# Lakonik/SSDNeRF

Measured on NVIDIA H100. Metric: rays/sec (128^2 render) & DDIM triplanes/sec, higher is better.
Workload: dtype fp16 tensor-core UNet (fp32 accumulate), fp32 renderer

## Files before the change

### ssdnerf_b200/csrc/conv_row2.cu

```cuda
#include "common.cuh"
#include "tc_common.cuh"
#include "conv_row_epilogue.cuh"
#include "../../include/ssdnerf_b200.h"
#include <cuda_fp16.h>

namespace ssdnerf {
using namespace tc;

constexpr int kRwThreads = 384;
constexpr int kRwRowSlot = 17 * 1024;
constexpr int kRwBSlot = kRwN * 128;
constexpr int kRwRows = 6, kRwBStages = 6;
constexpr int kGnMaxC = 384;
constexpr size_t kRwSmem = (size_t)kRwRows * kRwRowSlot + (size_t)kRwBStages * kRwBSlot + 1024  + 256  +
                           256  + 512 ;

struct ConvRowParams {
    uint32_t B, H;
    const __half* x1; uint32_t C1;
    const __half* x2; uint32_t C2;
    long long xs1[3], xs2[3];
    const float2* coef;
    const float* bias;
    const __half* residual;
    __half* out;
    float* qstats;
};

template <bool GN>
__global__ void __launch_bounds__(kRwThreads, 1)
k_conv_row2(const __grid_constant__ CUtensorMap mapB, const ConvRowParams p) {
    extern __shared__ uint8_t smem_raw[];
    uint8_t* smem = reinterpret_cast<uint8_t*>(((uintptr_t)smem_raw + 1023) & ~(uintptr_t)1023);
    uint8_t* sR = smem;
    uint8_t* sB = smem + kRwRows * kRwRowSlot;
    uint64_t* fullR = reinterpret_cast<uint64_t*>(sB + kRwBStages * kRwBSlot);
    uint64_t* emptyR = fullR + kRwRows;
    uint64_t* fullB = emptyR + kRwRows;
    uint64_t* emptyB = fullB + kRwBStages;
    float* qacc = reinterpret_cast<float*>(reinterpret_cast<uint8_t*>(fullR) + 256);
    float* sbias = qacc + 64;

    const int warp = threadIdx.x >> 5, lane = threadIdx.x & 31, wg = warp >> 2;
    const uint32_t tiles_per_img = p.H / 2, total_tiles = p.B * tiles_per_img;
    const uint32_t kc1 = p.C1 / 64, KC = (p.C1 + p.C2) / 64;
    const uint32_t tile0 = blockIdx.x, tstep = gridDim.x;
    const uint32_t my_tiles = tile0 < total_tiles ? (total_tiles - tile0 + tstep - 1) / tstep : 0;

    if (threadIdx.x == 0) {
        prefetch_tmap(&mapB);
        for (int i = 0; i < kRwRows; ++i) { mbar_init(&fullR[i], 4); mbar_init(&emptyR[i], 8); }
        for (int i = 0; i < kRwBStages; ++i) { mbar_init(&fullB[i], 1); mbar_init(&emptyB[i], 8); }
        fence_mbar_init();
    }
    for (int i = threadIdx.x; i < 64; i += kRwThreads) qacc[i] = 0.0f;
    for (int i = threadIdx.x; i < kRwN; i += kRwThreads) sbias[i] = p.bias ? __ldg(p.bias + i) : 0.0f;
    __syncthreads();
    pdl_trigger();
    pdl_wait();

    if (wg == 2) {
        setmaxnreg_dec<120>();
        const uint32_t lt = threadIdx.x - 256u;
        const uint32_t c8 = lt & 7u, p0 = lt >> 3;
        const uint32_t C = p.C1 + p.C2;
        uint32_t idx = 0;
        for (uint32_t tile = tile0; tile < total_tiles; tile += tstep) {
            const uint32_t b = tile / tiles_per_img, y0 = (tile - b * tiles_per_img) * 2;
            for (uint32_t j = 0; j < KC; ++j) {
                const bool first = j < kc1;
                const __half* src = first ? p.x1 : p.x2;
                const long long xs0 = first ? p.xs1[0] : p.xs2[0], xs1 = first ? p.xs1[1] : p.xs2[1], xs2 = first ? p.xs1[2] : p.xs2[2];
                const uint32_t cl = (first ? j : j - kc1) * 64u + c8 * 8u;
                float ca[8], cb[8];
                if (GN) {
                    const float4* cp = reinterpret_cast<const float4*>(p.coef + (size_t)b * C + j * 64u + c8 * 8u);
#pragma unroll
                    for (int k = 0; k < 4; ++k) {
                        const float4 t = __ldg(cp + k);
                        ca[2 * k] = 0.5f * t.x; cb[2 * k] = 0.5f * t.y; ca[2 * k + 1] = 0.5f * t.z; cb[2 * k + 1] = 0.5f * t.w;
                    }
                }
                for (uint32_t r = 0; r < 4; ++r) {
                    const int y = (int)(y0 + r) - 1;
                    const bool row_ok = y >= 0 && y < (int)p.H;
                    const __half* rowp = src + (long long)b * xs2 + (long long)(row_ok ? y : 0) * xs1 + cl;
                    uint4 v[9];
#pragma unroll
                    for (int n = 0; n < 9; ++n) {
                        const int x = (int)(p0 + 16u * n) - 1;
                        v[n] = (row_ok && (unsigned)x < (unsigned)kRwW) ? __ldg(reinterpret_cast<const uint4*>(rowp + (long long)x * xs0))
                                                                       : make_uint4(0, 0, 0, 0);
                    }
                    const uint32_t slot = idx % kRwRows;
                    mbar_wait(&emptyR[slot], ((idx / kRwRows) & 1u) ^ 1u);
                    const uint32_t dst = smem_u32(sR + slot * kRwRowSlot);
#pragma unroll
                    for (int n = 0; n < 9; ++n) {
                        const uint32_t px = p0 + 16u * n;
                        if (px >= 130u) continue;
                        uint4 o = v[n];
                        if (GN) {
                            const bool ok = row_ok && (unsigned)((int)px - 1) < (unsigned)kRwW;
                            const __half2* h = reinterpret_cast<const __half2*>(&v[n]);
                            uint32_t* ow = reinterpret_cast<uint32_t*>(&o);
#pragma unroll
                            for (int k = 0; k < 4; ++k) {
                                const float2 tt = __half22float2(h[k]);
                                const __half2 hh = __floats2half2_rn(fmaf(tt.x, ca[2 * k], cb[2 * k]), fmaf(tt.y, ca[2 * k + 1], cb[2 * k + 1]));
                                uint32_t hv = *reinterpret_cast<const uint32_t*>(&hh), tv;
                                asm("tanh.approx.f16x2 %0, %1;" : "=r"(tv) : "r"(hv));
                                const __half2 yy = __hfma2(hh, *reinterpret_cast<const __half2*>(&tv), hh);
                                ow[k] = ok ? *reinterpret_cast<const uint32_t*>(&yy) : 0u;
                            }
                        }
                        sts128(dst + px * 128u + ((c8 ^ (px & 7u)) << 4), o);
                    }
                    __syncwarp();
                    if (lane == 0) mbar_arrive(&fullR[slot]);
                    ++idx;
                }
            }
        }
    } else {
        setmaxnreg_inc<192>();
        const uint32_t a = (uint32_t)wg, wq = (uint32_t)warp & 3u, cq = (uint32_t)lane & 3u;
        const uint32_t steps_per_tile = KC * 9u, total_steps = my_tiles * steps_per_tile;
        auto issue_w = [&](uint32_t L) {
            const uint32_t s = L % kRwBStages;
            if (L >= (uint32_t)kRwBStages) mbar_wait(&emptyB[s], ((L / kRwBStages) - 1u) & 1u);
            mbar_expect_tx(&fullB[s], (uint32_t)kRwBSlot);
            const uint32_t rem = L % steps_per_tile;
            tma_load_4d(sB + s * kRwBSlot, &mapB, &fullB[s], (int)((rem / 9u) * 64u), 0, (int)(rem % 9u), 0);
        };
        if (threadIdx.x == 0)
            for (uint32_t L = 0; L < total_steps && L < (uint32_t)kRwBStages; ++L) issue_w(L);
        auto release_row = [&](uint32_t ring) { if (lane == 0) mbar_arrive(&emptyR[ring % kRwRows]); };
        uint32_t m = 0, ridx = 0;
        const uint32_t lrow = wq * 16u + ((uint32_t)lane & 15u);
        const uint32_t lk = (uint32_t)lane >> 4;
        for (uint32_t tile = tile0; tile < total_tiles; tile += tstep) {
            const uint32_t b = tile / tiles_per_img, y0 = (tile - b * tiles_per_img) * 2;
            float acc0[64], acc1[64];
#pragma unroll
            for (int i = 0; i < 64; ++i) { acc0[i] = 0.0f; acc1[i] = 0.0f; }
            for (uint32_t j = 0; j < KC; ++j) {
                const uint32_t unused = ridx + (a == 0 ? 3u : 0u);
                if (a == 1) { mbar_wait(&fullR[unused % kRwRows], (unused / kRwRows) & 1u); release_row(unused); }
                for (uint32_t ky = 0; ky < 3; ++ky) {
                    const uint32_t ring = ridx + ky + a;
                    mbar_wait(&fullR[ring % kRwRows], (ring / kRwRows) & 1u);
                    const uint32_t rowS = smem_u32(sR + (ring % kRwRows) * kRwRowSlot);
                    for (uint32_t kx = 0; kx < 3; ++kx) {
                        const uint32_t sb = m % kRwBStages;
                        uint32_t af[2][4][4];
#pragma unroll
                        for (uint32_t h = 0; h < 2; ++h) {
                            const uint32_t px = 64u * h + lrow + kx;
#pragma unroll
                            for (uint32_t k = 0; k < 4; ++k) ldmatrix_x4(rowS + px * 128u + (((2u * k + lk) ^ (px & 7u)) << 4), af[h][k]);
                        }
                        if (kx == 2) release_row(ring);
                        mbar_wait(&fullB[sb], (m / kRwBStages) & 1u);
                        const uint64_t b_desc = make_desc_sw128(smem_u32(sB + sb * kRwBSlot));
                        wgmma_fence();
                        fence_regs(acc0); fence_regs(acc1);
#pragma unroll
                        for (uint32_t k = 0; k < 4; ++k) {
                            wgmma_rs_n128(acc0, af[0][k], b_desc + 2 * k, 1u);
                            wgmma_rs_n128(acc1, af[1][k], b_desc + 2 * k, 1u);
                        }
                        wgmma_commit();
                        wgmma_wait<0>();
                        fence_regs(acc0); fence_regs(acc1);
                        if (lane == 0) mbar_arrive(&emptyB[sb]);
                        if (threadIdx.x == 0 && m >= 1 && m - 1 + kRwBStages < total_steps) issue_w(m - 1 + kRwBStages);
                        ++m;
                    }
                }
                if (a == 0) { mbar_wait(&fullR[unused % kRwRows], (unused / kRwRows) & 1u); release_row(unused); }
                ridx += 4;
            }
            const size_t pix0 = ((size_t)b * p.H + y0 + a) * kRwW;
#pragma unroll
            for (int i = 0; i < 16; ++i) {
                const uint32_t ch = 8u * i + 2u * cq;
                const float b0 = sbias[ch], b1 = sbias[ch + 1];
                float su = 0.0f, sq = 0.0f;
#pragma unroll
                for (int h = 0; h < 2; ++h) {
#pragma unroll
                    for (int hh = 0; hh < 2; ++hh) {
                        const size_t o = (pix0 + 64u * h + wq * 16u + ((uint32_t)lane >> 2) + 8u * hh) * kRwN + ch;
                        float v0 = (h ? acc1 : acc0)[4 * i + 2 * hh] + b0, v1 = (h ? acc1 : acc0)[4 * i + 2 * hh + 1] + b1;
                        if (p.residual) { const float2 r = __half22float2(*reinterpret_cast<const __half2*>(p.residual + o)); v0 += r.x; v1 += r.y; }
                        *reinterpret_cast<__half2*>(p.out + o) = __floats2half2_rn(v0, v1);
                        su += v0 + v1; sq = fmaf(v0, v0, fmaf(v1, v1, sq));
                    }
                }
                if (p.qstats) {
                    frag_quad_reduce(su, sq);
                    if ((lane & ~2) == 0) { float* qa = qacc + (2 * i + (lane >> 1)) * 2; atomicAdd(qa, su); atomicAdd(qa + 1, sq); }
                }
            }
            if (p.qstats) {
                asm volatile("bar.sync 1, 256;" ::: "memory");
                if (threadIdx.x < 64) {
                    const float val = qacc[threadIdx.x];
                    if (val != 0.0f) atomicAdd(p.qstats + (size_t)b * 64 + threadIdx.x, val);
                    qacc[threadIdx.x] = 0.0f;
                }
                asm volatile("bar.sync 1, 256;" ::: "memory");
            }
        }
    }
    __syncthreads();
}

__global__ void k_gn_coef(const float* __restrict__ q1, uint32_t C1, const float* __restrict__ q2, uint32_t C2, uint32_t HW,
                          const float* __restrict__ gamma, const float* __restrict__ beta, const float* __restrict__ scale_shift,
                          long long ss_batch_stride, float eps, float2* __restrict__ coef) {
    pdl_trigger();
    pdl_wait();
    __shared__ float2 s_mr[32];
    const uint32_t b = blockIdx.x, C = C1 + C2, cpg = C / 32u;
    const float inv_n = 1.0f / ((float)HW * (float)cpg);
    if (threadIdx.x < 32u) {
        const uint32_t q1n = C1 / 4, q2n = C2 / 4, nq = cpg / 4;
        float sm = 0.0f, sq = 0.0f;
        for (uint32_t i = 0; i < nq; ++i) {
            const uint32_t qi = threadIdx.x * nq + i;
            const float2 t = __ldg(reinterpret_cast<const float2*>(qi < q1n ? q1 + ((size_t)b * q1n + qi) * 2 : q2 + ((size_t)b * q2n + (qi - q1n)) * 2));
            sm += t.x; sq += t.y;
        }
        const float mean = sm * inv_n;
        s_mr[threadIdx.x] = make_float2(mean, rsqrtf(fmaxf(sq * inv_n - mean * mean, 0.0f) + eps));
    }
    __syncthreads();
    const float* ss = scale_shift ? scale_shift + (size_t)b * ss_batch_stride : nullptr;
    for (uint32_t c = threadIdx.x; c < C; c += blockDim.x) {
        const float2 mr = s_mr[c / cpg];
        const float ak = mr.y * __ldg(gamma + c);
        const float bk = __ldg(beta + c) - mr.x * ak;
        const float sc = ss ? 1.0f + __ldg(ss + c) : 1.0f, sh = ss ? __ldg(ss + C + c) : 0.0f;
        coef[(size_t)b * C + c] = make_float2(ak * sc, fmaf(bk, sc, sh));
    }
}

int make_map_4d_box(CUtensorMap* m, const void* base, uint64_t K, uint64_t e1, uint64_t e2, uint64_t e3, uint64_t s1, uint64_t s2, uint64_t s3,
                    uint32_t x1, uint32_t x2, uint32_t x3);

template <bool GN>
static int launch_row2(const CUtensorMap& mB, const ConvRowParams& p, int sms, cudaStream_t stream) {
    static DeviceOnce attr;
    if (attr.first()) {
        SSDNERF_CUDA_OK(cudaFuncSetAttribute(k_conv_row2<GN>, cudaFuncAttributeMaxDynamicSharedMemorySize, (int)kRwSmem));
    }
    const uint32_t total = p.B * (p.H / 2);
    SSDNERF_CUDA_OK(launch_pdl(k_conv_row2<GN>, dim3(total < (uint32_t)sms ? total : (uint32_t)sms), dim3(kRwThreads), kRwSmem, stream, mB, p));
    SSDNERF_LAUNCH_OK();
    return 0;
}

int conv_row2_launch(const ssdnerf_gemm_args* a, int sms, cudaStream_t stream) {
    if (((uintptr_t)a->a1 & 15u) || ((a->a1_strides[0] | a->a1_strides[1] | a->a1_strides[2]) & 15u) ||
        (a->a2 && (((uintptr_t)a->a2 & 15u) || ((a->a2_strides[0] | a->a2_strides[1] | a->a2_strides[2]) & 15u))) ||
        ((uintptr_t)a->out & 3u) || ((uintptr_t)a->residual & 3u))
        return set_error_msg(SSDNERF_ERR_ARG, "gemm: row-pair convolution needs 16-byte aligned inputs and strides, 4-byte aligned output / residual");
    ConvRowParams p{};
    p.B = a->d3; p.H = a->d2;
    p.x1 = (const __half*)a->a1; p.C1 = a->k1;
    p.x2 = (const __half*)a->a2; p.C2 = a->a2 ? a->k2 : 0;
    for (int i = 0; i < 3; ++i) { p.xs1[i] = (long long)(a->a1_strides[i] / 2); p.xs2[i] = a->a2 ? (long long)(a->a2_strides[i] / 2) : 0; }
    p.bias = a->bias_n; p.residual = (const __half*)a->residual; p.out = (__half*)a->out; p.qstats = a->qstats;
    const uint64_t ktot = (uint64_t)a->k1 + (a->a2 ? a->k2 : 0);
    CUtensorMap mB;
    if (int e = make_map_4d_box(&mB, a->b, ktot, a->n_rows_b ? a->n_rows_b : a->n, a->bx2 ? a->bx2 : 1, a->bx3 ? a->bx3 : 1, a->b_strides[0],
                                a->b_strides[1], a->b_strides[2], kRwN, 1, 1)) return e;
    return launch_row2<false>(mB, p, sms, stream);
}

}

using namespace ssdnerf;

extern "C" int ssdnerf_conv3x3_gn_f16(const ssdnerf_conv_gn_args* a, void* stream_) {
    cudaStream_t stream = (cudaStream_t)stream_;
    if (!a || !a->x1 || !a->q1 || !a->gamma || !a->beta || !a->w || !a->out || !a->coef_workspace)
        return set_error_msg(SSDNERF_ERR_ARG, "conv3x3_gn: x1, q1, gamma, beta, w, out and coef_workspace are required");
    if (a->B == 0 || a->H == 0) return 0;
    if (a->H % 2) return set_error_msg(SSDNERF_ERR_ARG, "conv3x3_gn: H must be even (tiles are row pairs)");
    if (a->C1 == 0 || a->C1 % 64 || a->C2 % 64 || (a->x2 && !a->q2)) return set_error_msg(SSDNERF_ERR_ARG, "conv3x3_gn: channel counts must be multiples of 64; x2 needs q2");
    const uint32_t C = a->C1 + (a->x2 ? a->C2 : 0);
    if (C > (uint32_t)kGnMaxC || (C / 32) % 4) return set_error_msg(SSDNERF_ERR_ARG, "conv3x3_gn: at most 384 input channels, channels per group a multiple of 4");
    if (a->w_rows < 128) return set_error_msg(SSDNERF_ERR_ARG, "conv3x3_gn: packed weight needs >= 128 rows per tap");
    if (((uintptr_t)a->x1 | (uintptr_t)a->x2 | (uintptr_t)a->out | (uintptr_t)a->residual | (uintptr_t)a->w | (uintptr_t)a->coef_workspace) & 15u)
        return set_error_msg(SSDNERF_ERR_ARG, "conv3x3_gn: tensors must be 16-byte aligned");
    ConvRowParams p{};
    p.B = a->B; p.H = a->H; p.x1 = (const __half*)a->x1; p.C1 = a->C1; p.x2 = (const __half*)a->x2; p.C2 = a->x2 ? a->C2 : 0;
    p.xs1[0] = p.C1; p.xs1[1] = (long long)kRwW * p.C1; p.xs1[2] = (long long)p.H * kRwW * p.C1;
    p.xs2[0] = p.C2; p.xs2[1] = (long long)kRwW * p.C2; p.xs2[2] = (long long)p.H * kRwW * p.C2;
    p.coef = (const float2*)a->coef_workspace; p.bias = a->bias; p.residual = (const __half*)a->residual; p.out = (__half*)a->out; p.qstats = a->qstats;
    int dev = 0, sms = 0;
    SSDNERF_CUDA_OK(cudaGetDevice(&dev));
    SSDNERF_CUDA_OK(cudaDeviceGetAttribute(&sms, cudaDevAttrMultiProcessorCount, dev));
    SSDNERF_CUDA_OK(launch_pdl(k_gn_coef, dim3(a->B), dim3(128), 0, stream, a->q1, a->C1, a->x2 ? a->q2 : (const float*)nullptr, p.C2, a->H * 128u,
                               a->gamma, a->beta, a->scale_shift, a->ss_batch_stride, a->eps, (float2*)a->coef_workspace));
    SSDNERF_LAUNCH_OK();
    CUtensorMap mB;
    if (int e = make_map_4d_box(&mB, a->w, C, a->w_rows, 9, 1, (uint64_t)C * 2, (uint64_t)a->w_rows * C * 2, (uint64_t)9 * a->w_rows * C * 2,
                                kRwN, 1, 1)) return e;
    return launch_row2<true>(mB, p, sms, stream);
}
```

### ssdnerf_b200/csrc/conv_row_epilogue.cuh

```cuda
#pragma once
#include "common.cuh"

namespace ssdnerf {

constexpr int kRwW = 128, kRwN = 128;

__device__ __forceinline__ void frag_quad_reduce(float& su, float& sq) {
    su += __shfl_xor_sync(0xffffffffu, su, 1); sq += __shfl_xor_sync(0xffffffffu, sq, 1);
#pragma unroll
    for (int m = 4; m <= 16; m <<= 1) { su += __shfl_xor_sync(0xffffffffu, su, m); sq += __shfl_xor_sync(0xffffffffu, sq, m); }
}

}
```

### ssdnerf_b200/csrc/gemm_tc.cu

```cuda
#include "common.cuh"
#include "tc_common.cuh"
#include "conv_row_epilogue.cuh"
#include "../../include/ssdnerf_b200.h"
#include <cuda_fp16.h>
#include <cstdio>

namespace ssdnerf {
using namespace tc;

constexpr int kGemmThreads = 384;
constexpr int kMaxBiasN = 2048;
constexpr int kBM = 128, kBK = 64;
constexpr int kABytes = kBM * kBK * 2;

struct GemmParams {
    uint32_t b1, b2, b3;
    uint32_t d1, d2, d3;
    uint32_t T1, T2, T3;
    uint32_t tiles_n;
    uint32_t taps;
    int8_t tap_ox[9], tap_oy[9];
    uint32_t a_stride;
    uint32_t kc1, kc2;
    uint32_t n_valid;
// ... 169 lines not shown
                        }
                    }
                    if (p.out_f32) {
                        float* op = reinterpret_cast<float*>(p.out) + o;
                        if (p.vec2 && okc1) *reinterpret_cast<float2*>(op) = make_float2(v0, v1);
                        else { op[0] = v0; if (okc1) op[1] = v1; }
                    } else {
                        __half* op = reinterpret_cast<__half*>(p.out) + o;
                        if (p.vec2 && okc1) *reinterpret_cast<__half2*>(op) = __floats2half2_rn(v0, v1);
                        else { op[0] = __float2half_rn(v0); if (okc1) op[1] = __float2half_rn(v1); }
                    }
                    if (!okc1) v1 = 0.0f;
                    su += v0 + v1; sq = fmaf(v0, v0, fmaf(v1, v1, sq));
                }
                if (p.qstats) {
                    frag_quad_reduce(su, sq);
                    if ((lane & ~2) == 0) {
                        float* qa = qacc + (slot * (BN / 4) + 2 * i + (lane >> 1)) * 2;
                        atomicAdd(qa, su); atomicAdd(qa + 1, sq);
                    }
                }
            }
            if (p.qstats) {
                asm volatile("bar.sync 1, 256;" ::: "memory");
                const uint32_t et = threadIdx.x - 128;
                const uint32_t nq = p.n_valid / 4;
                for (uint32_t i = et; i < (uint32_t)BN; i += 256) {
                    const float val = qacc[i];
                    const uint32_t sl = i / (BN / 2), qd = (i % (BN / 2)) >> 1, st = i & 1u;
                    const uint32_t gq = n_tile * (BN / 4) + qd;
                    if (val != 0.0f && gq < nq) atomicAdd(p.qstats + ((size_t)(img0 + sl) * nq + gq) * 2 + st, val);
                    qacc[i] = 0.0f;
                }
                asm volatile("bar.sync 1, 256;" ::: "memory");
            }
        }
        if (p.prof && threadIdx.x == 128) { atomicAdd(p.prof + 2, (unsigned long long)wf); atomicAdd(p.prof + 4, (unsigned long long)(clock64() - ct0)); }
    }
    __syncthreads();
    if (CL > 1) cluster_sync_all();
}

typedef CUresult (*PFN_encodeTiled)(CUtensorMap*, CUtensorMapDataType, cuuint32_t, void*, const cuuint64_t*, const cuuint64_t*,
                                    const cuuint32_t*, const cuuint32_t*, CUtensorMapInterleave, CUtensorMapSwizzle,
                                    CUtensorMapL2promotion, CUtensorMapFloatOOBfill);

static PFN_encodeTiled get_encode() {
    static PFN_encodeTiled fn = nullptr;
    if (!fn) {
        void* p = nullptr;
        cudaDriverEntryPointQueryResult qres;
        if (cudaGetDriverEntryPoint("cuTensorMapEncodeTiled", &p, cudaEnableDefault, &qres) != cudaSuccess || !p) return nullptr;
        fn = (PFN_encodeTiled)p;
    }
    return fn;
}

static int make_map_4d(CUtensorMap* m, const void* base, uint64_t K, uint64_t e1, uint64_t e2, uint64_t e3, uint64_t s1, uint64_t s2,
                       uint64_t s3, uint32_t x1, uint32_t x2, uint32_t x3, uint32_t trav = 1) {
    PFN_encodeTiled enc = get_encode();
    if (!enc) return set_error_msg(SSDNERF_ERR_CUDA, "cuTensorMapEncodeTiled entry point not found");
    if (((uintptr_t)base & 15u) || (s1 & 15u) || (s2 & 15u) || (s3 & 15u))
        return set_error_msg(SSDNERF_ERR_ARG, "gemm: TMA operands need 16-byte aligned base and strides");
    cuuint64_t dims[4] = {K, e1, e2, e3};
    cuuint64_t strides[3] = {s1, s2, s3};
    cuuint32_t box[4] = {64, x1 * trav, x2 * trav, x3};
    cuuint32_t estr[4] = {1, trav, trav, 1};
    const CUresult r = enc(m, CU_TENSOR_MAP_DATA_TYPE_FLOAT16, 4, const_cast<void*>(base), dims, strides, box, estr,
                           CU_TENSOR_MAP_INTERLEAVE_NONE, CU_TENSOR_MAP_SWIZZLE_128B, CU_TENSOR_MAP_L2_PROMOTION_L2_256B,
                           CU_TENSOR_MAP_FLOAT_OOB_FILL_NONE);
    if (r != CUDA_SUCCESS) {
        char buf[200];
        snprintf(buf, sizeof(buf), "cuTensorMapEncodeTiled failed (%d): dims {%llu,%llu,%llu,%llu} box {64,%u,%u,%u}", (int)r,
                 (unsigned long long)K, (unsigned long long)e1, (unsigned long long)e2, (unsigned long long)e3, x1, x2, x3);
        return set_error_msg(SSDNERF_ERR_CUDA, buf);
    }
    return 0;
}

int make_map_4d_box(CUtensorMap* m, const void* base, uint64_t K, uint64_t e1, uint64_t e2, uint64_t e3, uint64_t s1, uint64_t s2, uint64_t s3,
                    uint32_t x1, uint32_t x2, uint32_t x3) {
    return make_map_4d(m, base, K, e1, e2, e3, s1, s2, s3, x1, x2, x3);
}
int conv_row2_launch(const ssdnerf_gemm_args* a, int sms, cudaStream_t stream);

template <int BN, int CL>
static int launch_gemm(const CUtensorMap& mA1, const CUtensorMap& mA2, const CUtensorMap& mB, const GemmParams& p, int sms,
                       cudaStream_t stream) {
    using Cfg = GemmCfg<BN, CL>;
    static DeviceOnce attr;
    if (attr.first()) {
        SSDNERF_CUDA_OK(cudaFuncSetAttribute(k_gemm_tc<BN, CL>, cudaFuncAttributeMaxDynamicSharedMemorySize, (int)Cfg::kSmem));
    }
    const uint32_t tiles_m = p.T1 * p.T2 * p.T3;
    const uint32_t total = ((tiles_m + CL - 1) / CL) * p.tiles_n;
    cudaLaunchConfig_t cfg{};
    cfg.blockDim = dim3(kGemmThreads);
    cfg.dynamicSmemBytes = Cfg::kSmem;
    cfg.stream = stream;
    cudaLaunchAttribute at[2];
    at[0].id = cudaLaunchAttributeClusterDimension;
    at[0].val.clusterDim.x = CL; at[0].val.clusterDim.y = 1; at[0].val.clusterDim.z = 1;
    at[1].id = cudaLaunchAttributeProgrammaticStreamSerialization;
    at[1].val.programmaticStreamSerializationAllowed = pdl_enabled() ? 1 : 0;
    cfg.attrs = at; cfg.numAttrs = 2;
    static int max_clusters_dev[64] = {};
    int& max_clusters_cached = max_clusters_dev[current_device()];
    if (!max_clusters_cached) {
        max_clusters_cached = sms / CL;
        if (CL > 1) {
            cfg.gridDim = dim3((uint32_t)(sms / CL) * CL);
            int n = 0;
            cfg.numAttrs = 1;
            if (cudaOccupancyMaxActiveClusters(&n, k_gemm_tc<BN, CL>, &cfg) == cudaSuccess && n > 0 && n < max_clusters_cached) max_clusters_cached = n;
            cfg.numAttrs = 2;
            (void)cudaGetLastError();
        }
    }
    const uint32_t max_clusters = (uint32_t)max_clusters_cached;
    const uint32_t clusters = total < max_clusters ? total : max_clusters;
    cfg.gridDim = dim3(clusters * CL);
    SSDNERF_CUDA_OK(cudaLaunchKernelEx(&cfg, k_gemm_tc<BN, CL>, mA1, mA2, mB, p));
    SSDNERF_LAUNCH_OK();
    return 0;
}

}

using namespace ssdnerf;

extern "C" int ssdnerf_gemm_f16(const ssdnerf_gemm_args* a, void* stream_) {
    cudaStream_t stream = (cudaStream_t)stream_;
    if (!a || !a->a1 || !a->b || !a->out) return set_error_msg(SSDNERF_ERR_ARG, "gemm: a1, b and out are required");
    if (a->k1 == 0 || a->k1 % 64 || a->k2 % 64) return set_error_msg(SSDNERF_ERR_ARG, "gemm: K extents must be multiples of 64");
    if (a->b1 * a->b2 * a->b3 != 128) return set_error_msg(SSDNERF_ERR_ARG, "gemm: b1*b2*b3 must be 128");
    if (a->taps < 1 || a->taps > 9) return set_error_msg(SSDNERF_ERR_ARG, "gemm: taps must be in [1, 9]");
    if (a->taps != 1 && a->taps != 9 && !a->tap_offsets) return set_error_msg(SSDNERF_ERR_ARG, "gemm: taps other than 1 / 9 need tap_offsets");
    if (a->taps > 1 && a->b_batched) return set_error_msg(SSDNERF_ERR_ARG, "gemm: conv taps and batched B are exclusive");
    if (a->a_stride > 2) return set_error_msg(SSDNERF_ERR_ARG, "gemm: a_stride must be 0 / 1 / 2");
    const uint32_t a_stride = a->a_stride == 2 ? 2u : 1u;
    if (a_stride == 2 && (a->b1 * 2 > 256 || a->b2 * 2 > 256)) return set_error_msg(SSDNERF_ERR_ARG, "gemm: stride-2 boxes exceed the 256-element TMA limit");
    if (a->n == 0 || a->d1 == 0 || a->d2 == 0 || a->d3 == 0) return 0;
    int dev = 0, sms = 0;
    SSDNERF_CUDA_OK(cudaGetDevice(&dev));
    SSDNERF_CUDA_OK(cudaDeviceGetAttribute(&sms, cudaDevAttrMultiProcessorCount, dev));
    if (a->algo != 1 && a->taps == 9 && !a->tap_offsets && a_stride == 1 && a->d1 == 128 && a->b1 == 128 && a->b2 == 1 && a->b3 == 1 && a->n == 128 && !a->out_f32 && !a->b_batched &&
        (a->d2 % 2) == 0 && a->alpha == 1.0f && (a->bn == 0 || a->bn == 128) && a->cluster <= 1 && a->so1 == 128 && a->so2 == 128 * 128 &&
        a->so3 == (long long)a->d2 * 128 * 128 && (!a->qstats || a->stats_hw == 0) && (a->n_rows_b == 0 || a->n_rows_b >= 128))
        return ssdnerf::conv_row2_launch(a, sms, stream);
    if (a->algo == 2) return set_error_msg(SSDNERF_ERR_ARG, "gemm: algo 2 (row-pair convolution) needs taps 9, 128-pixel rows, 128 output channels, fp16 output");
    int bn = (int)a->bn;
    if (!bn) {
        const uint32_t tiles_m = div_up(a->d1, a->b1) * div_up(a->d2, a->b2) * div_up(a->d3, a->b3);
        double best = 1e30;
        const int cand[3] = {256, 128, 64};
        const double eff[3] = {1.0, 0.80, 0.50};
        for (int i = 0; i < 3; ++i) {
            if (cand[i] > 64 && (uint32_t)cand[i] / 2 >= a->n) continue;
            const uint32_t tiles = tiles_m * div_up(a->n, (uint32_t)cand[i]);
            const double t = (double)div_up(tiles, (uint32_t)sms) * cand[i] / eff[i];
            if (t < best) { best = t; bn = cand[i]; }
        }
    }
    if (bn != 64 && bn != 128 && bn != 256) return set_error_msg(SSDNERF_ERR_ARG, "gemm: bn must be 64, 128 or 256");

    GemmParams p{};
    p.b1 = a->b1; p.b2 = a->b2; p.b3 = a->b3; p.d1 = a->d1; p.d2 = a->d2; p.d3 = a->d3;
    p.T1 = div_up(a->d1, a->b1); p.T2 = div_up(a->d2, a->b2); p.T3 = div_up(a->d3, a->b3);
    p.tiles_n = div_up(a->n, (uint32_t)bn);
    p.a_stride = a_stride;
    for (uint32_t t = 0; t < 9; ++t) {
        if (a->tap_offsets) { p.tap_ox[t] = a->tap_offsets[2 * t]; p.tap_oy[t] = a->tap_offsets[2 * t + 1]; }
        else if (a->taps == 9) { p.tap_ox[t] = (int8_t)((int)(t % 3) - 1); p.tap_oy[t] = (int8_t)((int)(t / 3) - 1); }
        else { p.tap_ox[t] = 0; p.tap_oy[t] = 0; }
    }
    p.taps = a->taps; p.kc1 = a->k1 / 64; p.kc2 = a->a2 ? a->k2 / 64 : 0; p.n_valid = a->n; p.b_batched = a->b_batched;
    p.alpha = a->alpha; p.bias_n = a->bias_n; p.residual = (const __half*)a->residual; p.out = a->out; p.out_f32 = a->out_f32;
    p.so1 = a->so1; p.so2 = a->so2; p.so3 = a->so3;
    p.qstats = a->qstats; p.stats_hw = a->stats_hw; p.prof = (unsigned long long*)a->debug_cycles;
    const uintptr_t pair_align = a->out_f32 ? 8u : 4u;
    p.vec2 = ((a->so1 | a->so2 | a->so3) & 1) == 0 && ((uintptr_t)a->out % pair_align) == 0 && ((uintptr_t)a->residual & 3u) == 0;
    if (a->bias_n && a->n > (uint32_t)kMaxBiasN) return set_error_msg(SSDNERF_ERR_ARG, "gemm: bias vectors longer than 2048 are not supported");
    if (a->qstats && (a->n % 4)) return set_error_msg(SSDNERF_ERR_ARG, "gemm: quad statistics need n % 4 == 0");
    if (a->qstats && !a->stats_hw && a->b3 > 2) return set_error_msg(SSDNERF_ERR_ARG, "gemm: fused quad statistics cover at most 2 images per 128-row tile (b3 <= 2)");
    if (a->qstats && a->stats_hw && (a->stats_hw % 64)) return set_error_msg(SSDNERF_ERR_ARG, "gemm: stats_hw must be a multiple of 64");
    const uint64_t ktot = (uint64_t)a->k1 + (a->a2 ? a->k2 : 0);

    CUtensorMap mA1, mA2, mB;
    const uint64_t e1 = (uint64_t)a->d1 * a_stride, e2 = (uint64_t)a->d2 * a_stride;
    if (int e = make_map_4d(&mA1, a->a1, a->k1, e1, e2, a->d3, a->a1_strides[0], a->a1_strides[1], a->a1_strides[2], a->b1, a->b2, a->b3, a_stride)) return e;
    if (a->a2) {
        if (int e = make_map_4d(&mA2, a->a2, a->k2, e1, e2, a->d3, a->a2_strides[0], a->a2_strides[1], a->a2_strides[2], a->b1, a->b2, a->b3, a_stride)) return e;
    } else {
        mA2 = mA1;
    }
    int cl = 1;
    if ((a->cluster == 2 || a->cluster == 4 || a->cluster == 8) && !a->b_batched && bn >= 128) cl = (int)a->cluster;
    if (int e = make_map_4d(&mB, a->b, ktot, a->n_rows_b ? a->n_rows_b : a->n, a->bx2 ? a->bx2 : 1, a->bx3 ? a->bx3 : 1, a->b_strides[0],
                            a->b_strides[1], a->b_strides[2], (uint32_t)(bn / cl), 1, 1)) return e;

    if (bn == 256) {
        if (cl == 8) return launch_gemm<256, 8>(mA1, mA2, mB, p, sms, stream);
        if (cl == 4) return launch_gemm<256, 4>(mA1, mA2, mB, p, sms, stream);
        return cl == 2 ? launch_gemm<256, 2>(mA1, mA2, mB, p, sms, stream) : launch_gemm<256, 1>(mA1, mA2, mB, p, sms, stream);
    }
    if (bn == 128) {
        if (cl == 8) return launch_gemm<128, 8>(mA1, mA2, mB, p, sms, stream);
        if (cl == 4) return launch_gemm<128, 4>(mA1, mA2, mB, p, sms, stream);
        return cl == 2 ? launch_gemm<128, 2>(mA1, mA2, mB, p, sms, stream) : launch_gemm<128, 1>(mA1, mA2, mB, p, sms, stream);
    }
    return launch_gemm<64, 1>(mA1, mA2, mB, p, sms, stream);
}
```

### ssdnerf_b200/unet_ops.py

```python
import ctypes

import torch

from . import _lib as N

c_u64 = ctypes.c_uint64
c_ll = ctypes.c_longlong


class GemmArgs(ctypes.Structure):
    _fields_ = [
        ('a1', N.c_void_p), ('a1_strides', c_u64 * 3), ('k1', N.c_u32),
        ('a2', N.c_void_p), ('a2_strides', c_u64 * 3), ('k2', N.c_u32),
        ('d1', N.c_u32), ('d2', N.c_u32), ('d3', N.c_u32), ('b1', N.c_u32), ('b2', N.c_u32), ('b3', N.c_u32),
        ('taps', N.c_u32),
        ('b', N.c_void_p), ('b_strides', c_u64 * 3), ('n', N.c_u32), ('n_rows_b', N.c_u32), ('bx2', N.c_u32), ('bx3', N.c_u32),
        ('b_batched', N.c_u32),
        ('bn', N.c_u32), ('cluster', N.c_u32), ('alpha', N.c_f32), ('bias_n', N.c_void_p), ('residual', N.c_void_p),
        ('out', N.c_void_p), ('out_f32', N.c_u32), ('so1', c_ll), ('so2', c_ll), ('so3', c_ll),
        ('qstats', N.c_void_p), ('stats_hw', N.c_u32), ('debug_cycles', N.c_void_p), ('algo', N.c_u32),
        ('tap_offsets', N.c_void_p), ('a_stride', N.c_u32),
    ]


GEMM_PROF = None
GEMM_LOG = None


def _launch(a):
    if GEMM_PROF is not None:
        a.debug_cycles = GEMM_PROF.data_ptr()
    if GEMM_LOG is not None:
        GEMM_LOG.append(dict(M=int(a.d1) * int(a.d2) * int(a.d3), N=int(a.n), K=int(a.k1) + int(a.k2), taps=int(a.taps), bn=int(a.bn),
                             cluster=int(a.cluster), batched=int(a.b_batched), qstats=bool(a.qstats), f32=int(a.out_f32)))
    N.check(N.lib().ssdnerf_gemm_f16(ctypes.byref(a), N.stream_ptr()))


def _pad_rows(w, mult=64):
    n = w.shape[-2]
    pad = (-n) % mult
    if pad:
        w = torch.cat([w, w.new_zeros(*w.shape[:-2], pad, w.shape[-1])], dim=-2)
    return w


def pack_linear_weight(w):
    w = w.detach().reshape(w.shape[0], -1).half()
    assert w.shape[1] % 64 == 0, 'K must be a multiple of 64'
    return _pad_rows(w).contiguous()


def pack_conv_weight(w, cin_pad=None):
    cout, cin = w.shape[0], w.shape[1]
    cin_pad = cin_pad or ((cin + 63) // 64 * 64)
    wp = w.detach().permute(2, 3, 0, 1).reshape(9, cout, cin).half()
    if cin_pad != cin:
        wp = torch.cat([wp, wp.new_zeros(9, cout, cin_pad - cin)], dim=-1)
    return _pad_rows(wp).contiguous()


def linear_f16(a, w, bias=None, residual=None, out=None, out_f32=False, alpha=1.0, bn=0, n=None, cluster=0, qstats=None, stats_hw=0):
    N.require_cuda(a, w)
    M, K = a.shape
    n = n if n is not None else w.shape[0]
    if out is None:
        out = torch.empty(M, n, dtype=torch.float32 if out_f32 else torch.float16, device=a.device)
    g = GemmArgs()
    g.a1, g.k1 = a.data_ptr(), K
    rs = a.stride(0) * 2
    g.a1_strides = (c_u64 * 3)(rs, rs * M, rs * M)
    g.d1, g.d2, g.d3, g.b1, g.b2, g.b3 = M, 1, 1, 128, 1, 1
    g.taps = 1
    g.b, g.n, g.n_rows_b, g.bx2, g.bx3 = w.data_ptr(), n, w.shape[0], 1, 1
    ws = w.stride(0) * 2
    g.b_strides = (c_u64 * 3)(ws, ws * w.shape[0], ws * w.shape[0])
    g.bn, g.alpha, g.cluster = bn, alpha, cluster
    g.bias_n = bias.data_ptr() if bias is not None else None
    g.residual = residual.data_ptr() if residual is not None else None
    g.out, g.out_f32 = out.data_ptr(), int(out.dtype == torch.float32)
    g.so1, g.so2, g.so3 = out.stride(0), 0, 0
    if qstats is not None:
        g.qstats, g.stats_hw = qstats.data_ptr(), stats_hw
    _launch(g)
    return out


def _conv_boxes(H, W):
    bw = min(W, 128)
    bh = min(H, 128 // bw)
    nb = 128 // (bw * bh)
    return bw, bh, nb


def conv3x3_f16(x, wp, cout, bias=None, x2=None, residual=None, out=None, out_f32=False, taps=9, bn=0, cluster=0, qstats=None, algo=0):
    N.require_cuda(x, wp)
    B, H, W, C1 = x.shape
    C2 = x2.shape[-1] if x2 is not None else 0
    assert x.is_contiguous() and (x2 is None or x2.is_contiguous())
    assert wp.shape[-1] == C1 + C2 and C1 % 64 == 0 and C2 % 64 == 0, (wp.shape, C1, C2)
    if out is None:
        out = torch.empty(B, H, W, cout, dtype=torch.float32 if out_f32 else torch.float16, device=x.device)
    bw, bh, nb = _conv_boxes(H, W)
    g = GemmArgs()
    g.a1, g.k1 = x.data_ptr(), C1
    g.a1_strides = (c_u64 * 3)(C1 * 2, W * C1 * 2, H * W * C1 * 2)
    if x2 is not None:
        g.a2, g.k2 = x2.data_ptr(), C2
        g.a2_strides = (c_u64 * 3)(C2 * 2, W * C2 * 2, H * W * C2 * 2)
    g.d1, g.d2, g.d3, g.b1, g.b2, g.b3 = W, H, B, bw, bh, nb
    g.taps = taps
    ktot = C1 + C2
    rows = wp.shape[-2]
    g.b, g.n, g.n_rows_b, g.bx2, g.bx3 = wp.data_ptr(), cout, rows, taps, 1
    g.b_strides = (c_u64 * 3)(ktot * 2, rows * ktot * 2, taps * rows * ktot * 2)
    g.bn, g.alpha, g.cluster, g.algo = bn, 1.0, cluster, algo
    g.bias_n = bias.data_ptr() if bias is not None else None
    g.residual = residual.data_ptr() if residual is not None else None
# ... 320 lines not shown
```

Measured before the change: 97.61 million.

## Generalize row convolution kernel to 64/32-pixel rows and multiple output-channel blocks

Templates the row-pair 3x3 convolution kernel on row width W, so each warpgroup covers 128/W rows and the smem row ring is sized per width. It adds output-channel blocking, which extends the row-conv path to 64- and 32-wide feature maps and to N up to 1024. Dispatch now defaults to this path for W=64 with N=256 and small K, where the generic implicit GEMM was used before. The new indexing for multi-row tiles, the extra staged rows and the larger bias buffer add complexity, and the loader batches two rows when W<128.

```diff
diff --git a/ssdnerf_b200/csrc/conv_row2.cu b/ssdnerf_b200/csrc/conv_row2.cu
--- a/ssdnerf_b200/csrc/conv_row2.cu
+++ b/ssdnerf_b200/csrc/conv_row2.cu
@@ -8,15 +8,28 @@
 using namespace tc;
 
 constexpr int kRwThreads = 384;
-constexpr int kRwRowSlot = 17 * 1024;
 constexpr int kRwBSlot = kRwN * 128;
-constexpr int kRwRows = 6, kRwBStages = 6;
+constexpr int kRwBStages = 6;
 constexpr int kGnMaxC = 384;
-constexpr size_t kRwSmem = (size_t)kRwRows * kRwRowSlot + (size_t)kRwBStages * kRwBSlot + 1024  + 256  +
-                           256  + 512 ;
+
+template <int W>
+struct RowCfg {
+    static constexpr int kRowsWg = 128 / W;
+    static constexpr int kStaged = 2 * kRowsWg + 2;
+    static constexpr int kPx = W + 2;
+    static constexpr int kRowSlot = (kPx * 128 + 1023) / 1024 * 1024;
+    static constexpr int kRing = kStaged + 2;
+    static constexpr int kNP = (kPx + 15) / 16;
+    static constexpr int kLB = W == 128 ? 1 : 2;
+    static constexpr size_t kSmem = (size_t)kRing * kRowSlot + (size_t)kRwBStages * kRwBSlot + 1024  + 512  +
+                                    256  + kRwMaxN * 4 ;
+    static_assert(kStaged % kLB == 0, "loader batches must tile the staged rows");
+    static_assert(kSmem <= 227 * 1024, "shared memory");
+};
 
 struct ConvRowParams {
     uint32_t B, H;
+    uint32_t n;
     const __half* x1; uint32_t C1;
     const __half* x2; uint32_t C2;
     long long xs1[3], xs2[3];
@@ -27,34 +40,37 @@
     float* qstats;
 };
 
-template <bool GN>
+template <bool GN, int W>
 __global__ void __launch_bounds__(kRwThreads, 1)
-k_conv_row2(const __grid_constant__ CUtensorMap mapB, const ConvRowParams p) {
+k_conv_row(const __grid_constant__ CUtensorMap mapB, const ConvRowParams p) {
+    using Cfg = RowCfg<W>;
+    constexpr uint32_t kRowsWg = Cfg::kRowsWg, kStaged = Cfg::kStaged, kRing = Cfg::kRing, kRowSlot = Cfg::kRowSlot;
     extern __shared__ uint8_t smem_raw[];
     uint8_t* smem = reinterpret_cast<uint8_t*>(((uintptr_t)smem_raw + 1023) & ~(uintptr_t)1023);
     uint8_t* sR = smem;
-    uint8_t* sB = smem + kRwRows * kRwRowSlot;
+    uint8_t* sB = smem + kRing * kRowSlot;
     uint64_t* fullR = reinterpret_cast<uint64_t*>(sB + kRwBStages * kRwBSlot);
-    uint64_t* emptyR = fullR + kRwRows;
-    uint64_t* fullB = emptyR + kRwRows;
+    uint64_t* emptyR = fullR + kRing;
+    uint64_t* fullB = emptyR + kRing;
     uint64_t* emptyB = fullB + kRwBStages;
-    float* qacc = reinterpret_cast<float*>(reinterpret_cast<uint8_t*>(fullR) + 256);
+    float* qacc = reinterpret_cast<float*>(reinterpret_cast<uint8_t*>(fullR) + 512);
     float* sbias = qacc + 64;
 
     const int warp = threadIdx.x >> 5, lane = threadIdx.x & 31, wg = warp >> 2;
-    const uint32_t tiles_per_img = p.H / 2, total_tiles = p.B * tiles_per_img;
+    const uint32_t nblocks = p.n / kRwN, groups = p.H / (2 * kRowsWg);
+    const uint32_t total_tiles = p.B * groups * nblocks;
     const uint32_t kc1 = p.C1 / 64, KC = (p.C1 + p.C2) / 64;
     const uint32_t tile0 = blockIdx.x, tstep = gridDim.x;
     const uint32_t my_tiles = tile0 < total_tiles ? (total_tiles - tile0 + tstep - 1) / tstep : 0;
 
     if (threadIdx.x == 0) {
         prefetch_tmap(&mapB);
-        for (int i = 0; i < kRwRows; ++i) { mbar_init(&fullR[i], 4); mbar_init(&emptyR[i], 8); }
+        for (int i = 0; i < (int)kRing; ++i) { mbar_init(&fullR[i], 4); mbar_init(&emptyR[i], 8); }
         for (int i = 0; i < kRwBStages; ++i) { mbar_init(&fullB[i], 1); mbar_init(&emptyB[i], 8); }
         fence_mbar_init();
     }
     for (int i = threadIdx.x; i < 64; i += kRwThreads) qacc[i] = 0.0f;
-    for (int i = threadIdx.x; i < kRwN; i += kRwThreads) sbias[i] = p.bias ? __ldg(p.bias + i) : 0.0f;
+    for (uint32_t i = threadIdx.x; i < p.n; i += kRwThreads) sbias[i] = p.bias ? __ldg(p.bias + i) : 0.0f;
     __syncthreads();
     pdl_trigger();
     pdl_wait();
@@ -66,7 +82,7 @@
         const uint32_t C = p.C1 + p.C2;
         uint32_t idx = 0;
         for (uint32_t tile = tile0; tile < total_tiles; tile += tstep) {
-            const uint32_t b = tile / tiles_per_img, y0 = (tile - b * tiles_per_img) * 2;
+            const uint32_t bg = tile / nblocks, b = bg / groups, y0 = (bg - b * groups) * (2 * kRowsWg);
             for (uint32_t j = 0; j < KC; ++j) {
                 const bool first = j < kc1;
                 const __half* src = first ? p.x1 : p.x2;
@@ -81,44 +97,51 @@
                         ca[2 * k] = 0.5f * t.x; cb[2 * k] = 0.5f * t.y; ca[2 * k + 1] = 0.5f * t.z; cb[2 * k + 1] = 0.5f * t.w;
                     }
                 }
-                for (uint32_t r = 0; r < 4; ++r) {
-                    const int y = (int)(y0 + r) - 1;
-                    const bool row_ok = y >= 0 && y < (int)p.H;
-                    const __half* rowp = src + (long long)b * xs2 + (long long)(row_ok ? y : 0) * xs1 + cl;
-                    uint4 v[9];
-#pragma unroll
-                    for (int n = 0; n < 9; ++n) {
-                        const int x = (int)(p0 + 16u * n) - 1;
-                        v[n] = (row_ok && (unsigned)x < (unsigned)kRwW) ? __ldg(reinterpret_cast<const uint4*>(rowp + (long long)x * xs0))
-                                                                       : make_uint4(0, 0, 0, 0);
-                    }
-                    const uint32_t slot = idx % kRwRows;
-                    mbar_wait(&emptyR[slot], ((idx / kRwRows) & 1u) ^ 1u);
-                    const uint32_t dst = smem_u32(sR + slot * kRwRowSlot);
-#pragma unroll
-                    for (int n = 0; n < 9; ++n) {
-                        const uint32_t px = p0 + 16u * n;
-                        if (px >= 130u) continue;
-                        uint4 o = v[n];
-                        if (GN) {
-                            const bool ok = row_ok && (unsigned)((int)px - 1) < (unsigned)kRwW;
-                            const __half2* h = reinterpret_cast<const __half2*>(&v[n]);
-                            uint32_t* ow = reinterpret_cast<uint32_t*>(&o);
-#pragma unroll
-                            for (int k = 0; k < 4; ++k) {
-                                const float2 tt = __half22float2(h[k]);
-                                const __half2 hh = __floats2half2_rn(fmaf(tt.x, ca[2 * k], cb[2 * k]), fmaf(tt.y, ca[2 * k + 1], cb[2 * k + 1]));
-                                uint32_t hv = *reinterpret_cast<const uint32_t*>(&hh), tv;
-                                asm("tanh.approx.f16x2 %0, %1;" : "=r"(tv) : "r"(hv));
-                                const __half2 yy = __hfma2(hh, *reinterpret_cast<const __half2*>(&tv), hh);
-                                ow[k] = ok ? *reinterpret_cast<const uint32_t*>(&yy) : 0u;
+                for (uint32_t r0 = 0; r0 < kStaged; r0 += Cfg::kLB) {
+                    uint4 v[Cfg::kLB][Cfg::kNP];
+                    bool row_ok[Cfg::kLB];
+#pragma unroll
+                    for (int rr = 0; rr < Cfg::kLB; ++rr) {
+                        const int y = (int)(y0 + r0 + rr) - 1;
+                        row_ok[rr] = y >= 0 && y < (int)p.H;
+                        const __half* rowp = src + (long long)b * xs2 + (long long)(row_ok[rr] ? y : 0) * xs1 + cl;
+#pragma unroll
+                        for (int n = 0; n < Cfg::kNP; ++n) {
+                            const int x = (int)(p0 + 16u * n) - 1;
+                            v[rr][n] = (row_ok[rr] && (unsigned)x < (unsigned)W) ? __ldg(reinterpret_cast<const uint4*>(rowp + (long long)x * xs0))
+                                                                                 : make_uint4(0, 0, 0, 0);
+                        }
+                    }
+#pragma unroll
+                    for (int rr = 0; rr < Cfg::kLB; ++rr) {
+                        const uint32_t slot = idx % kRing;
+                        mbar_wait(&emptyR[slot], ((idx / kRing) & 1u) ^ 1u);
+                        const uint32_t dst = smem_u32(sR + slot * kRowSlot);
+#pragma unroll
+                        for (int n = 0; n < Cfg::kNP; ++n) {
+                            const uint32_t px = p0 + 16u * n;
+                            if (px >= (uint32_t)Cfg::kPx) continue;
+                            uint4 o = v[rr][n];
+                            if (GN) {
+                                const bool ok = row_ok[rr] && (unsigned)((int)px - 1) < (unsigned)W;
+                                const __half2* h = reinterpret_cast<const __half2*>(&v[rr][n]);
+                                uint32_t* ow = reinterpret_cast<uint32_t*>(&o);
+#pragma unroll
+                                for (int k = 0; k < 4; ++k) {
+                                    const float2 tt = __half22float2(h[k]);
+                                    const __half2 hh = __floats2half2_rn(fmaf(tt.x, ca[2 * k], cb[2 * k]), fmaf(tt.y, ca[2 * k + 1], cb[2 * k + 1]));
+                                    uint32_t hv = *reinterpret_cast<const uint32_t*>(&hh), tv;
+                                    asm("tanh.approx.f16x2 %0, %1;" : "=r"(tv) : "r"(hv));
+                                    const __half2 yy = __hfma2(hh, *reinterpret_cast<const __half2*>(&tv), hh);
+                                    ow[k] = ok ? *reinterpret_cast<const uint32_t*>(&yy) : 0u;
+                                }
                             }
-                        }
-                        sts128(dst + px * 128u + ((c8 ^ (px & 7u)) << 4), o);
-                    }
-                    __syncwarp();
-                    if (lane == 0) mbar_arrive(&fullR[slot]);
-                    ++idx;
+                            sts128(dst + px * 128u + ((c8 ^ (px & 7u)) << 4), o);
+                        }
+                        __syncwarp();
+                        if (lane == 0) mbar_arrive(&fullR[slot]);
+                        ++idx;
+                    }
                 }
             }
         }
@@ -130,37 +153,45 @@
             const uint32_t s = L % kRwBStages;
             if (L >= (uint32_t)kRwBStages) mbar_wait(&emptyB[s], ((L / kRwBStages) - 1u) & 1u);
             mbar_expect_tx(&fullB[s], (uint32_t)kRwBSlot);
-            const uint32_t rem = L % steps_per_tile;
-            tma_load_4d(sB + s * kRwBSlot, &mapB, &fullB[s], (int)((rem / 9u) * 64u), 0, (int)(rem % 9u), 0);
+            const uint32_t rem = L % steps_per_tile, nb = (tile0 + (L / steps_per_tile) * tstep) % nblocks;
+            tma_load_4d(sB + s * kRwBSlot, &mapB, &fullB[s], (int)((rem / 9u) * 64u), (int)(nb * kRwN), (int)(rem % 9u), 0);
         };
         if (threadIdx.x == 0)
             for (uint32_t L = 0; L < total_steps && L < (uint32_t)kRwBStages; ++L) issue_w(L);
-        auto release_row = [&](uint32_t ring) { if (lane == 0) mbar_arrive(&emptyR[ring % kRwRows]); };
+        auto release_row = [&](uint32_t ring) { if (lane == 0) mbar_arrive(&emptyR[ring % kRing]); };
+        auto wait_row = [&](uint32_t ring) { mbar_wait(&fullR[ring % kRing], (ring / kRing) & 1u); };
         uint32_t m = 0, ridx = 0;
         const uint32_t lrow = wq * 16u + ((uint32_t)lane & 15u);
         const uint32_t lk = (uint32_t)lane >> 4;
         for (uint32_t tile = tile0; tile < total_tiles; tile += tstep) {
-            const uint32_t b = tile / tiles_per_img, y0 = (tile - b * tiles_per_img) * 2;
+            const uint32_t bg = tile / nblocks, nb = tile - bg * nblocks, b = bg / groups, y0 = (bg - b * groups) * (2 * kRowsWg);
             float acc0[64], acc1[64];
 #pragma unroll
             for (int i = 0; i < 64; ++i) { acc0[i] = 0.0f; acc1[i] = 0.0f; }
             for (uint32_t j = 0; j < KC; ++j) {
-                const uint32_t unused = ridx + (a == 0 ? 3u : 0u);
-                if (a == 1) { mbar_wait(&fullR[unused % kRwRows], (unused / kRwRows) & 1u); release_row(unused); }
+                const uint32_t unused = ridx + (a == 0 ? kRowsWg + 2u : 0u);
+                if (a == 1)
+                    for (uint32_t r = 0; r < kRowsWg; ++r) { wait_row(unused + r); release_row(unused + r); }
+                const uint32_t base = ridx + a * kRowsWg;
                 for (uint32_t ky = 0; ky < 3; ++ky) {
-                    const uint32_t ring = ridx + ky + a;
-                    mbar_wait(&fullR[ring % kRwRows], (ring / kRwRows) & 1u);
-                    const uint32_t rowS = smem_u32(sR + (ring % kRwRows) * kRwRowSlot);
+                    for (uint32_t r = 0; r < kRowsWg; ++r) wait_row(base + ky + r);
+                    uint32_t rowS[2];
+#pragma unroll
+                    for (uint32_t h = 0; h < 2; ++h) rowS[h] = smem_u32(sR + ((base + ky + (64u * h + lrow) / W) % kRing) * kRowSlot);
                     for (uint32_t kx = 0; kx < 3; ++kx) {
                         const uint32_t sb = m % kRwBStages;
                         uint32_t af[2][4][4];
 #pragma unroll
                         for (uint32_t h = 0; h < 2; ++h) {
-                            const uint32_t px = 64u * h + lrow + kx;
-#pragma unroll
-                            for (uint32_t k = 0; k < 4; ++k) ldmatrix_x4(rowS + px * 128u + (((2u * k + lk) ^ (px & 7u)) << 4), af[h][k]);
-                        }
-                        if (kx == 2) release_row(ring);
+                            const uint32_t px = (64u * h + lrow) % W + kx;
+#pragma unroll
+                            for (uint32_t k = 0; k < 4; ++k) ldmatrix_x4(rowS[h] + px * 128u + (((2u * k + lk) ^ (px & 7u)) << 4), af[h][k]);
+                        }
+                        if (kx == 2) {
+                            release_row(base + ky);
+                            if (ky == 2)
+                                for (uint32_t r = 3; r <= kRowsWg + 1; ++r) release_row(base + r);
+                        }
                         mbar_wait(&fullB[sb], (m / kRwBStages) & 1u);
                         const uint64_t b_desc = make_desc_sw128(smem_u32(sB + sb * kRwBSlot));
                         wgmma_fence();
@@ -178,22 +209,24 @@
                         ++m;
                     }
                 }
-                if (a == 0) { mbar_wait(&fullR[unused % kRwRows], (unused / kRwRows) & 1u); release_row(unused); }
-                ridx += 4;
+                if (a == 0)
+                    for (uint32_t r = 0; r < kRowsWg; ++r) { wait_row(unused + r); release_row(unused + r); }
+                ridx += kStaged;
             }
-            const size_t pix0 = ((size_t)b * p.H + y0 + a) * kRwW;
+            const size_t pix0 = ((size_t)b * p.H + y0 + a * kRowsWg) * W;
+            const uint32_t c0 = nb * kRwN;
 #pragma unroll
             for (int i = 0; i < 16; ++i) {
-                const uint32_t ch = 8u * i + 2u * cq;
+                const uint32_t ch = c0 + 8u * i + 2u * cq;
                 const float b0 = sbias[ch], b1 = sbias[ch + 1];
                 float su = 0.0f, sq = 0.0f;
 #pragma unroll
                 for (int h = 0; h < 2; ++h) {
 #pragma unroll
                     for (int hh = 0; hh < 2; ++hh) {
-                        const size_t o = (pix0 + 64u * h + wq * 16u + ((uint32_t)lane >> 2) + 8u * hh) * kRwN + ch;
+                        const size_t o = (pix0 + 64u * h + wq * 16u + ((uint32_t)lane >> 2) + 8u * hh) * p.n + ch;
                         float v0 = (h ? acc1 : acc0)[4 * i + 2 * hh] + b0, v1 = (h ? acc1 : acc0)[4 * i + 2 * hh + 1] + b1;
-                        if (p.residual) { const float2 r = __half22float2(*reinterpret_cast<const __half2*>(p.residual + o)); v0 += r.x; v1 += r.y; }
+                        if (p.residual) { const float2 r = __half22float2(__ldg(reinterpret_cast<const __half2*>(p.residual + o))); v0 += r.x; v1 += r.y; }
                         *reinterpret_cast<__half2*>(p.out + o) = __floats2half2_rn(v0, v1);
                         su += v0 + v1; sq = fmaf(v0, v0, fmaf(v1, v1, sq));
                     }
@@ -207,7 +240,7 @@
                 asm volatile("bar.sync 1, 256;" ::: "memory");
                 if (threadIdx.x < 64) {
                     const float val = qacc[threadIdx.x];
-                    if (val != 0.0f) atomicAdd(p.qstats + (size_t)b * 64 + threadIdx.x, val);
+                    if (val != 0.0f) atomicAdd(p.qstats + (size_t)b * (p.n / 2) + nb * 64u + threadIdx.x, val);
                     qacc[threadIdx.x] = 0.0f;
                 }
                 asm volatile("bar.sync 1, 256;" ::: "memory");
@@ -250,25 +283,26 @@
 int make_map_4d_box(CUtensorMap* m, const void* base, uint64_t K, uint64_t e1, uint64_t e2, uint64_t e3, uint64_t s1, uint64_t s2, uint64_t s3,
                     uint32_t x1, uint32_t x2, uint32_t x3);
 
-template <bool GN>
-static int launch_row2(const CUtensorMap& mB, const ConvRowParams& p, int sms, cudaStream_t stream) {
+template <bool GN, int W>
+static int launch_row(const CUtensorMap& mB, const ConvRowParams& p, int sms, cudaStream_t stream) {
+    constexpr size_t smem = RowCfg<W>::kSmem;
     static DeviceOnce attr;
     if (attr.first()) {
-        SSDNERF_CUDA_OK(cudaFuncSetAttribute(k_conv_row2<GN>, cudaFuncAttributeMaxDynamicSharedMemorySize, (int)kRwSmem));
-    }
-    const uint32_t total = p.B * (p.H / 2);
-    SSDNERF_CUDA_OK(launch_pdl(k_conv_row2<GN>, dim3(total < (uint32_t)sms ? total : (uint32_t)sms), dim3(kRwThreads), kRwSmem, stream, mB, p));
+        SSDNERF_CUDA_OK(cudaFuncSetAttribute(k_conv_row<GN, W>, cudaFuncAttributeMaxDynamicSharedMemorySize, (int)smem));
+    }
+    const uint32_t total = p.B * (p.H / (256 / W)) * (p.n / kRwN);
+    SSDNERF_CUDA_OK(launch_pdl(k_conv_row<GN, W>, dim3(total < (uint32_t)sms ? total : (uint32_t)sms), dim3(kRwThreads), smem, stream, mB, p));
     SSDNERF_LAUNCH_OK();
     return 0;
 }
 
-int conv_row2_launch(const ssdnerf_gemm_args* a, int sms, cudaStream_t stream) {
+int conv_row_launch(const ssdnerf_gemm_args* a, int sms, cudaStream_t stream) {
     if (((uintptr_t)a->a1 & 15u) || ((a->a1_strides[0] | a->a1_strides[1] | a->a1_strides[2]) & 15u) ||
         (a->a2 && (((uintptr_t)a->a2 & 15u) || ((a->a2_strides[0] | a->a2_strides[1] | a->a2_strides[2]) & 15u))) ||
         ((uintptr_t)a->out & 3u) || ((uintptr_t)a->residual & 3u))
-        return set_error_msg(SSDNERF_ERR_ARG, "gemm: row-pair convolution needs 16-byte aligned inputs and strides, 4-byte aligned output / residual");
+        return set_error_msg(SSDNERF_ERR_ARG, "gemm: row convolution needs 16-byte aligned inputs and strides, 4-byte aligned output / residual");
     ConvRowParams p{};
-    p.B = a->d3; p.H = a->d2;
+    p.B = a->d3; p.H = a->d2; p.n = a->n;
     p.x1 = (const __half*)a->a1; p.C1 = a->k1;
     p.x2 = (const __half*)a->a2; p.C2 = a->a2 ? a->k2 : 0;
     for (int i = 0; i < 3; ++i) { p.xs1[i] = (long long)(a->a1_strides[i] / 2); p.xs2[i] = a->a2 ? (long long)(a->a2_strides[i] / 2) : 0; }
@@ -277,7 +311,9 @@
     CUtensorMap mB;
     if (int e = make_map_4d_box(&mB, a->b, ktot, a->n_rows_b ? a->n_rows_b : a->n, a->bx2 ? a->bx2 : 1, a->bx3 ? a->bx3 : 1, a->b_strides[0],
                                 a->b_strides[1], a->b_strides[2], kRwN, 1, 1)) return e;
-    return launch_row2<false>(mB, p, sms, stream);
+    if (a->d1 == 64) return launch_row<false, 64>(mB, p, sms, stream);
+    if (a->d1 == 32) return launch_row<false, 32>(mB, p, sms, stream);
+    return launch_row<false, 128>(mB, p, sms, stream);
 }
 
 }
@@ -297,9 +333,10 @@
     if (((uintptr_t)a->x1 | (uintptr_t)a->x2 | (uintptr_t)a->out | (uintptr_t)a->residual | (uintptr_t)a->w | (uintptr_t)a->coef_workspace) & 15u)
         return set_error_msg(SSDNERF_ERR_ARG, "conv3x3_gn: tensors must be 16-byte aligned");
     ConvRowParams p{};
-    p.B = a->B; p.H = a->H; p.x1 = (const __half*)a->x1; p.C1 = a->C1; p.x2 = (const __half*)a->x2; p.C2 = a->x2 ? a->C2 : 0;
-    p.xs1[0] = p.C1; p.xs1[1] = (long long)kRwW * p.C1; p.xs1[2] = (long long)p.H * kRwW * p.C1;
-    p.xs2[0] = p.C2; p.xs2[1] = (long long)kRwW * p.C2; p.xs2[2] = (long long)p.H * kRwW * p.C2;
+    constexpr long long kW = 128;
+    p.B = a->B; p.H = a->H; p.n = kRwN; p.x1 = (const __half*)a->x1; p.C1 = a->C1; p.x2 = (const __half*)a->x2; p.C2 = a->x2 ? a->C2 : 0;
+    p.xs1[0] = p.C1; p.xs1[1] = kW * p.C1; p.xs1[2] = (long long)p.H * kW * p.C1;
+    p.xs2[0] = p.C2; p.xs2[1] = kW * p.C2; p.xs2[2] = (long long)p.H * kW * p.C2;
     p.coef = (const float2*)a->coef_workspace; p.bias = a->bias; p.residual = (const __half*)a->residual; p.out = (__half*)a->out; p.qstats = a->qstats;
     int dev = 0, sms = 0;
     SSDNERF_CUDA_OK(cudaGetDevice(&dev));
@@ -310,5 +347,5 @@
     CUtensorMap mB;
     if (int e = make_map_4d_box(&mB, a->w, C, a->w_rows, 9, 1, (uint64_t)C * 2, (uint64_t)a->w_rows * C * 2, (uint64_t)9 * a->w_rows * C * 2,
                                 kRwN, 1, 1)) return e;
-    return launch_row2<true>(mB, p, sms, stream);
-}
+    return launch_row<true, 128>(mB, p, sms, stream);
+}
diff --git a/ssdnerf_b200/csrc/conv_row_epilogue.cuh b/ssdnerf_b200/csrc/conv_row_epilogue.cuh
--- a/ssdnerf_b200/csrc/conv_row_epilogue.cuh
+++ b/ssdnerf_b200/csrc/conv_row_epilogue.cuh
@@ -3,7 +3,8 @@
 
 namespace ssdnerf {
 
-constexpr int kRwW = 128, kRwN = 128;
+constexpr int kRwN = 128;
+constexpr int kRwMaxN = 1024;
 
 __device__ __forceinline__ void frag_quad_reduce(float& su, float& sq) {
     su += __shfl_xor_sync(0xffffffffu, su, 1); sq += __shfl_xor_sync(0xffffffffu, sq, 1);
diff --git a/ssdnerf_b200/csrc/gemm_tc.cu b/ssdnerf_b200/csrc/gemm_tc.cu
--- a/ssdnerf_b200/csrc/gemm_tc.cu
+++ b/ssdnerf_b200/csrc/gemm_tc.cu
@@ -275,7 +275,7 @@
                     uint32_t x1, uint32_t x2, uint32_t x3) {
     return make_map_4d(m, base, K, e1, e2, e3, s1, s2, s3, x1, x2, x3);
 }
-int conv_row2_launch(const ssdnerf_gemm_args* a, int sms, cudaStream_t stream);
+int conv_row_launch(const ssdnerf_gemm_args* a, int sms, cudaStream_t stream);
 
 template <int BN, int CL>
 static int launch_gemm(const CUtensorMap& mA1, const CUtensorMap& mA2, const CUtensorMap& mB, const GemmParams& p, int sms,
@@ -337,11 +337,17 @@
     int dev = 0, sms = 0;
     SSDNERF_CUDA_OK(cudaGetDevice(&dev));
     SSDNERF_CUDA_OK(cudaDeviceGetAttribute(&sms, cudaDevAttrMultiProcessorCount, dev));
-    if (a->algo != 1 && a->taps == 9 && !a->tap_offsets && a_stride == 1 && a->d1 == 128 && a->b1 == 128 && a->b2 == 1 && a->b3 == 1 && a->n == 128 && !a->out_f32 && !a->b_batched &&
-        (a->d2 % 2) == 0 && a->alpha == 1.0f && (a->bn == 0 || a->bn == 128) && a->cluster <= 1 && a->so1 == 128 && a->so2 == 128 * 128 &&
-        a->so3 == (long long)a->d2 * 128 * 128 && (!a->qstats || a->stats_hw == 0) && (a->n_rows_b == 0 || a->n_rows_b >= 128))
-        return ssdnerf::conv_row2_launch(a, sms, stream);
-    if (a->algo == 2) return set_error_msg(SSDNERF_ERR_ARG, "gemm: algo 2 (row-pair convolution) needs taps 9, 128-pixel rows, 128 output channels, fp16 output");
+    const uint32_t W = a->d1;
+    const bool row_shape = (W == 128 || W == 64 || W == 32) && a->b1 == W && a->b2 == 128 / W && a->b3 == 1 && (a->d2 % (256 / W)) == 0;
+    const bool row_default = (W == 128 && a->n == 128) || (W == 64 && a->n == 256 && a->k1 + (a->a2 ? a->k2 : 0) <= 256);
+    if ((a->algo == 2 || (a->algo == 0 && row_default)) && a->taps == 9 && !a->tap_offsets && a_stride == 1 && row_shape && a->n % kRwN == 0 && a->n <= (uint32_t)kRwMaxN &&
+        !a->out_f32 && !a->b_batched && a->alpha == 1.0f && (a->bn == 0 || a->bn == 128) && a->cluster <= 1 && a->so1 == (long long)a->n &&
+        a->so2 == (long long)W * a->n && a->so3 == (long long)a->d2 * W * a->n && (!a->qstats || a->stats_hw == 0) &&
+        (a->n_rows_b == 0 || a->n_rows_b >= a->n))
+        return ssdnerf::conv_row_launch(a, sms, stream);
+    if (a->algo == 2)
+        return set_error_msg(SSDNERF_ERR_ARG, "gemm: algo 2 (row convolution) needs taps 9, stride 1, 128 / 64 / 32-pixel rows with the default boxes, "
+                                              "a multiple of 256 / W rows, output channels a multiple of 128 (at most 1024), fp16 dense output");
     int bn = (int)a->bn;
     if (!bn) {
         const uint32_t tiles_m = div_up(a->d1, a->b1) * div_up(a->d2, a->b2) * div_up(a->d3, a->b3);
diff --git a/ssdnerf_b200/unet_ops.py b/ssdnerf_b200/unet_ops.py
--- a/ssdnerf_b200/unet_ops.py
+++ b/ssdnerf_b200/unet_ops.py
@@ -32,7 +32,9 @@
         a.debug_cycles = GEMM_PROF.data_ptr()
     if GEMM_LOG is not None:
         GEMM_LOG.append(dict(M=int(a.d1) * int(a.d2) * int(a.d3), N=int(a.n), K=int(a.k1) + int(a.k2), taps=int(a.taps), bn=int(a.bn),
-                             cluster=int(a.cluster), batched=int(a.b_batched), qstats=bool(a.qstats), f32=int(a.out_f32)))
+                             cluster=int(a.cluster), batched=int(a.b_batched), qstats=bool(a.qstats), f32=int(a.out_f32),
+                             d=(int(a.d1), int(a.d2), int(a.d3)), k1=int(a.k1), k2=int(a.k2) if a.a2 else 0, bias=bool(a.bias_n),
+                             residual=bool(a.residual), tap_offsets=bool(a.tap_offsets), a_stride=int(a.a_stride)))
     N.check(N.lib().ssdnerf_gemm_f16(ctypes.byref(a), N.stream_ptr()))
 
 
```

After: 97.59 million (median of 6 runs). About the same (-0.0%).
